# PimLb/POMDP_PBVI_Exploration

Hardware: AMD Instinct MI355X
Metric: alpha-vector backups/sec (higher is better)
Workload: dtype f32

## Files before the change

### pomdp_pbvi_exploration_amd/csrc/engine.hip

```cpp
#include <algorithm>
#include <cmath>
#include <cstdio>
#include <cstdlib>
#include <cstring>
#include <condition_variable>
#include <mutex>
#include <new>
#include <string>
#include <thread>
#include <unistd.h>
#include <vector>

#include "backup_kernels.h"

namespace pbvi {

static thread_local std::string g_err;
static int g_poison = -1;
static bool poison_enabled() {
    if (g_poison < 0) g_poison = getenv("PBVI_POISON") != nullptr ? 1 : 0;
    return g_poison == 1;
}
void set_error(const std::string& msg) { g_err = msg; }

#define HIPCHK(expr)                                                                         \
    do {                                                                                     \
        hipError_t _e = (expr);                                                              \
        if (_e != hipSuccess) {                                                              \
            set_error(std::string(#expr) + ": " + hipGetErrorString(_e));                    \
            (void)hipGetLastError();                                                         \
            return (_e == hipErrorOutOfMemory || _e == hipErrorMemoryAllocation) ? PBVI_ENOMEM : PBVI_ERUNTIME; \
        }                                                                                    \
    } while (0)

#define FAIL(code, msg)        \
    do {                       \
        set_error(msg);        \
        return (code);         \
    } while (0)

class CopyPool {
public:
    static CopyPool& get() {
        static CopyPool* pool = new CopyPool();
        return *pool;
    }
// ... 296 lines not shown
    for (int off = 32; off > 0; off >>= 1) {
        const int o = __shfl_xor(first, off, 64);
        first = o < first ? o : first;
    }
    if ((tid & 63) == 0) red[tid >> 6] = first;
    __syncthreads();
    if (tid == 0) {
        int m = red[0];
        for (int w = 1; w < 4; ++w) m = red[w] < m ? red[w] : m;
        key[b] = m == 0x7fffffff ? k_tiles : m;
    }
}

__global__ void k_rank_sort(const int32_t* __restrict__ key, int B, int32_t* __restrict__ perm) {
    const int lane = threadIdx.x & 63;
    const int i = blockIdx.x * 4 + (threadIdx.x >> 6);
    if (i >= B) return;
    const int ki = key[i];
    int rank = 0;
    for (int j = lane; j < B; j += 64) {
        const int kj = key[j];
        rank += (kj < ki || (kj == ki && j < i)) ? 1 : 0;
    }
#pragma unroll
    for (int off = 32; off > 0; off >>= 1) rank += __shfl_xor(rank, off, 64);
    if (lane == 0) perm[rank] = i;
}

__device__ __forceinline__ void tile_or_block(const uint8_t* __restrict__ flags, const int32_t* __restrict__ perm, int B, int k_tiles,
                                              uint8_t* __restrict__ nz, int bx, int tile);
template <typename T>
__global__ void k_gather_rows_v(const T* __restrict__ src, T* __restrict__ dst, int ld, const int32_t* __restrict__ perm,
                                const int32_t* __restrict__ ids, const uint8_t* __restrict__ flags = nullptr, int B = 0,
                                int k_tiles = 0, uint8_t* __restrict__ nz = nullptr, int or_rows = 0) {
    if ((int)blockIdx.y < or_rows) {
        if ((int)blockIdx.x * 64 < k_tiles) tile_or_block(flags, perm, B, k_tiles, nz, blockIdx.x, blockIdx.y);
        return;
    }
    constexpr int NS = 16 / (int)sizeof(T);
    typedef T TN __attribute__((ext_vector_type(NS)));
    const int c = blockIdx.x * 256 + threadIdx.x;
    if (c * NS >= ld) return;
    const int row = blockIdx.y - or_rows;
    int r = row;
    if (perm) r = perm[r];
    if (ids) r = ids[r];
    *(TN*)(dst + (int64_t)row * ld + (int64_t)c * NS) = *(const TN*)(src + (int64_t)r * ld + (int64_t)c * NS);
}

__device__ __forceinline__ void tile_or_block(const uint8_t* __restrict__ flags, const int32_t* __restrict__ perm, int B, int k_tiles,
                                              uint8_t* __restrict__ nz, int bx, int tile) {
    __shared__ uint32_t part[16][17];
    const int cw = threadIdx.x & 15, rs = threadIdx.x >> 4;
    const int kt0 = (bx * 16 + cw) * 4;
    const int r1 = (tile + 1) * 256 < B ? (tile + 1) * 256 : B;
    uint32_t f = 0;
    if (kt0 < k_tiles) {
        const bool whole = kt0 + 4 <= k_tiles && (k_tiles & 3) == 0;
#pragma unroll 4
        for (int r = tile * 256 + rs; r < r1; r += 16) {
            const uint8_t* p = flags + (int64_t)(perm ? perm[r] : r) * k_tiles + kt0;
            if (whole) {
                f |= *(const uint32_t*)p;
            } else {
                for (int e = 0; e < 4 && kt0 + e < k_tiles; ++e) f |= (uint32_t)p[e] << (8 * e);
            }
        }
    }
    part[rs][cw] = f;
    __syncthreads();
    if (rs == 0 && kt0 < k_tiles) {
        for (int x = 1; x < 16; ++x) f |= part[x][cw];
        for (int e = 0; e < 4 && kt0 + e < k_tiles; ++e) nz[(int64_t)tile * k_tiles + kt0 + e] = ((f >> (8 * e)) & 0xffu) ? 1 : 0;
    }
}

template <typename T>
__global__ void k_gather_rows(const T* __restrict__ src, T* __restrict__ dst, int ld, const int32_t* __restrict__ perm) {
    const int s = blockIdx.x * 256 + threadIdx.x;
    if (s >= ld) return;
// ... 190 lines not shown
};

template <typename T>
class EngineT : public EngineBase {
   public:
    static constexpr bool kF32 = sizeof(T) == 4;

    int device_ = 0;
    hipStream_t stream_ = nullptr;
    int S_ = 0, A_ = 0, O_ = 0, R_ = 0, S_pad_ = 0, mode_ = 0;
    int64_t bytes_ = 0;
    int64_t room() const {
        if (DevBuf::limit_bytes() >= 0) return DevBuf::limit_bytes() - bytes_;
        size_t fr = 0, tot = 0;
        if (hipMemGetInfo(&fr, &tot) != hipSuccess) {
            (void)hipGetLastError();
            return INT64_MAX;
        }
        return (int64_t)fr;
    }
    double tie_rel_user_ = -1.0;

    DevBuf rs_, rto_, er_, sup_;
    DevBuf alpha_, alpha_buf_, alpha_small_;
    std::vector<int32_t> prim_ids_;
    int64_t prim_off_ = 0;
    bool prim_valid_ = false, alpha_on_primary_ = false;
    uint64_t prim_layout_ver_ = 0;
    uint64_t screen_layout_seen_ = 0;
    int64_t screen_off_seen_ = 0;
    int64_t V_ = 0;
    DevBuf bel_;
    int64_t B_ = 0, B_pad_ = 0;
    DevBuf gam_, slabs_, best_v_, best_score_, err_, dead_, queue_, counters_, rdot_, action_, aqueue_, out_, keep_;
    DevBuf bv2_, bs2_, err2_, queue2_, prune_cnt_;
    DevBuf stage_, keys_, perm_, action_res_, best_res_;
    DevBuf rep_, uniq_, inv_, slot_, out_full_;
    DevBuf store_[2], ids_;
    int64_t store_rows_[2] = {0, 0};
    DevBuf in_ptr_, in_src_, bu_act_, bu_obs_, bu_row_, bu_unnorm_, bu_mass_, bu_out_, walk64_, rto64_;
    std::vector<int32_t> h_rs_;
    DevBuf btl_, btc_, val_exact_;
    DevBuf bp_, nzP_, pmag_, prd_;
    bool btl_valid_ = false;
    bool vmax_exact_ = true;
    DevBuf snz_, sbtl_, sbtc_;
    int64_t snz_rows_ = 0, sbt_rows_ = 0;
    int64_t walk_rows_ = 0;
    DevBuf vmax_bk_;
    bool have_bk_vmax_ = false;
    hipEvent_t walk_ev_[8] = {};
    void* host_stage_ = nullptr;
    size_t host_stage_cap_ = 0;
    DevBuf keys_tmp_, keys_act_, keys_best_, keys_rows_;
    DevBuf acand_;
    DevBuf rf_q2_, rf_q2p_, rf_q2d_;
    DevBuf rf_v_, rf_slot_, rf_sc_, rf_entry_, rf_n_, rf_tiles_, rf_ibv_, rf_ibi_, rf_cnt_, rf_W_, rf_Cx_, rf_nzW_, rf_klW_, rf_kcW_;
    int formulation_ = 0;
    int last_formulation_ = 1;
    int64_t f64_pairs_ = 0;
    const int32_t* res_action_ = nullptr;
    const int32_t* res_best_ = nullptr;
    int64_t res_unique_ = 0;
    bool full_valid_ = false;
    std::vector<int32_t> h_perm_;
    bool h_perm_valid_ = false;
// ... 36 lines not shown
    int64_t res_B_ = 0;
    int screen_mode_ = 1;
    int split_mode_ = 1;
    bool split_supported_ = false;
    int fuse_project_ = 1;
    double irr_frac_ = 0.0;
    DevBuf irr_;
    DevBuf mat_, vlist_;
    DevBuf ctile_;
    std::vector<int32_t> h_ctile_;
    int n_mat_ = 0;
    bool gam_pad_compact_ = false;
    std::vector<uint8_t> h_mat_;
    std::vector<int> h_vlist_;
    int64_t mat_V_ = -1;
    uint64_t dead_ver_ = 0;
    int64_t dead_pairs_ = 0, dead_count_ = 0;
    int* rf_counts_ = nullptr;
    bool last_deferred_nothing_ = false;
    bool owns_streams_ = true;
    EngineT<float>* screen_ = nullptr;
    std::vector<int32_t> h_reach_ref_;
    std::vector<double> h_rto_ref_, h_er_ref_;
    uint64_t alpha_ver_ = 1, bel_ver_ = 1;
    uint64_t screen_alpha_seen_ = 0, screen_bel_seen_ = 0;

    ~EngineT() override {
        (void)hipSetDevice(device_);
        if (screen_) {
            (void)hipStreamSynchronize(stream_);
            delete screen_;
            screen_ = nullptr;
        }
        DevBuf* all[] = {&rs_, &rto_, &er_, &sup_, &alpha_buf_, &alpha_small_, &bel_, &gam_, &slabs_, &best_v_, &best_score_, &err_,
                         &dead_, &queue_, &counters_, &rdot_, &action_, &aqueue_, &out_, &keep_, &bv2_, &bs2_,
                         &err2_, &queue2_, &prune_cnt_, &nzB_, &nzA_, &klist_, &kcount_, &nchunks_, &need_, &skws_, &stage_, &keys_, &perm_,
                         &action_res_, &best_res_, &rep_, &uniq_, &inv_, &slot_, &out_full_, &btl_, &btc_, &val_exact_, &store_[0], &store_[1], &ids_, &in_ptr_, &in_src_, &bu_act_, &bu_obs_,
                         &bu_unnorm_, &bu_mass_, &bu_out_, &bu_row_, &walk64_, &rto64_, &bp_, &nzP_, &pmag_, &prd_, &keys_tmp_, &keys_act_, &keys_best_, &keys_rows_, &rf_v_, &rf_slot_, &rf_sc_, &rf_entry_, &rf_n_, &rf_tiles_,
                         &snz_, &sbtl_, &sbtc_, &vmax_bk_, &rf_ibv_, &rf_ibi_, &rf_cnt_, &rf_W_, &rf_Cx_, &rf_nzW_, &rf_klW_, &rf_kcW_,
                         &dense_, &nzD_, &nzAlpha_, &prod_, &klistD_, &kcountD_, &nchunksD_, &mat_, &vlist_, &irr_, &rowflags_, &nzBw_, &scr_flag_, &ctile_, &acand_, &rf_q2_, &rf_q2p_, &rf_q2d_, &e_bv_, &e_bs_, &e_err_, &e_rdot_, &e_act_, &e_ares_, &e_bres_, &e_rep_, &e_uniq_, &e_inv_, &e_slotd_, &e_cnt_, &e_out_, &e_slot_};
        static const bool dbg = getenv("PBVI_DEBUG") != nullptr;
        auto chk = [&](hipError_t e, const char* what) {
            if (e != hipSuccess && dbg) fprintf(stderr, "[pbvi] engine teardown: %s: %s\n", what, hipGetErrorString(e));
        };
        for (auto& e : walk_ev_)
            if (e) chk(hipEventDestroy(e), "hipEventDestroy(walk)");
        for (DevBuf* b : all) b->release();
        if (host_stage_) chk(hipHostFree(host_stage_), "hipHostFree(stage)");
        if (ids_pin_) chk(hipHostFree(ids_pin_), "hipHostFree(ids)");
        if (h_flag_) chk(hipHostFree(h_flag_), "hipHostFree(flag)");
        if (kc_pin_) chk(hipHostFree(kc_pin_), "hipHostFree(kcount)");
        for (hipEvent_t& ev : ev_early_)
            if (ev) chk(hipEventDestroy(ev), "hipEventDestroy(early)");
        if (ev_ids_) chk(hipEventDestroy(ev_ids_), "hipEventDestroy(ids)");
        if (ev_nzA_) chk(hipEventDestroy(ev_nzA_), "hipEventDestroy(nzA)");
        for (auto& e : ev_)
            if (e) chk(hipEventDestroy(e), "hipEventDestroy(ev)");
        for (auto& e : ev_pg_)
            if (e) chk(hipEventDestroy(e), "hipEventDestroy(ev_pg)");
        if (ev_fork_) chk(hipEventDestroy(ev_fork_), "hipEventDestroy(fork)");
        if (ev_join_) chk(hipEventDestroy(ev_join_), "hipEventDestroy(join)");
        if (ev_lists_) chk(hipEventDestroy(ev_lists_), "hipEventDestroy(lists)");
        for (auto& e : ev_xr_)
            if (e) chk(hipEventDestroy(e), "hipEventDestroy(xr)");
        if (owns_streams_) {
            if (stream3_) chk(hipStreamDestroy(stream3_), "hipStreamDestroy(3)");
            if (stream2_) chk(hipStreamDestroy(stream2_), "hipStreamDestroy(2)");
// ... 257 lines not shown
                HIPCHK(hipMemcpyAsync(nb.p, alpha_.p, (size_t)V_ * S_pad_ * sizeof(T), hipMemcpyDeviceToDevice, stream_));
            HIPCHK(hipStreamSynchronize(stream_));
            bytes_ -= (int64_t)alpha_buf_.cap;
            alpha_buf_.release();
            alpha_buf_ = nb;
            alpha_view(alpha_buf_, 0);
        } else {
            HIPCHK(hipMemsetAsync(alpha_.as<T>() + (size_t)V_ * S_pad_, 0, (size_t)S_pad_ * sizeof(T), stream_));
        }
        prim_valid_ = alpha_on_primary_ = false;
        HIPCHK(hipMemcpy2DAsync(alpha_.as<T>() + (size_t)V_ * S_pad_, (size_t)S_pad_ * sizeof(T), alpha,
                                (size_t)S_ * sizeof(T), (size_t)S_ * sizeof(T), (size_t)n, hipMemcpyHostToDevice, stream_));
        V_ = Vn;
        ++alpha_ver_;
        int rc = refresh_magnitude_row();
        if (rc) return rc;
        HIPCHK(hipStreamSynchronize(stream_));
        have_result_ = false;
        return PBVI_OK;
    }

    int64_t alpha_count() const override { return V_; }

    int beliefs_finish(int64_t B, const T* src, const int32_t* src_ids) {
        const int64_t Bp = round_up(B, GEMM_BM);
        const int k_tiles = S_pad_ / GEMM_BK;
        int rc = bel_.ensure((size_t)Bp * S_pad_ * sizeof(T), &bytes_);
        if (rc) return rc;
        if ((rc = rowflags_.ensure((size_t)B * k_tiles, &bytes_))) return rc;
        if ((rc = keys_.ensure((size_t)B * sizeof(int32_t), &bytes_))) return rc;
        if ((rc = perm_.ensure((size_t)B * sizeof(int32_t), &bytes_))) return rc;
        if ((rc = nzA_.ensure((size_t)(Bp / GEMM_BM) * k_tiles, &bytes_))) return rc;
        if (Bp > B) HIPCHK(hipMemsetAsync(bel_.as<T>() + (size_t)B * S_pad_, 0, (size_t)(Bp - B) * S_pad_ * sizeof(T), stream_));
        static const bool no_sort = getenv("PBVI_NO_BELIEF_SORT") != nullptr;
        sorted_ = B > (kF32 ? GEMM_BM : 128) && !no_sort;
        hipLaunchKernelGGL(k_row_flags<T>, dim3((unsigned)B), dim3(256), 0, stream_, src, S_pad_, src_ids, S_pad_, k_tiles,
                           rowflags_.as<uint8_t>(), keys_.as<int32_t>());
        HIPCHK(hipGetLastError());
        const int32_t* perm = nullptr;
        if (sorted_) {
            hipLaunchKernelGGL(k_rank_sort, dim3((unsigned)((B + 3) / 4)), dim3(256), 0, stream_, keys_.as<int32_t>(), (int)B,
                               perm_.as<int32_t>());
            HIPCHK(hipGetLastError());
            perm = perm_.as<int32_t>();
        }
        constexpr int NS = 16 / (int)sizeof(T);
        const int or_rows = (int)(Bp / GEMM_BM);
        hipLaunchKernelGGL(k_gather_rows_v<T>, dim3((S_pad_ / NS + 255) / 256, (unsigned)(B + or_rows)), dim3(256), 0, stream_, src,
                           bel_.as<T>(), S_pad_, perm, src_ids, rowflags_.as<uint8_t>(), (int)B, k_tiles, nzA_.as<uint8_t>(), or_rows);
        HIPCHK(hipGetLastError());
        if (!ev_nzA_) HIPCHK(hipEventCreateWithFlags(&ev_nzA_, hipEventDisableTiming));
        HIPCHK(hipEventRecord(ev_nzA_, stream_));
        B_ = B;
        B_pad_ = Bp;
        ++bel_ver_;
        rowflags_ver_ = bel_ver_;
        nzA_ver_ = bel_ver_;
        h_perm_valid_ = false;
        have_result_ = false;
        btl_valid_ = false;
        return PBVI_OK;
    }

    int* pinned_flag() {
        if (!h_flag_ && hipHostMalloc((void**)&h_flag_, 128, hipHostMallocDefault) != hipSuccess) {
            (void)hipGetLastError();
            h_flag_ = nullptr;
        }
        return h_flag_;
    }

    int host_perm() {
        if (!sorted_ || h_perm_valid_) return PBVI_OK;
        h_perm_.resize((size_t)B_);
        HIPCHK(hipMemcpyAsync(h_perm_.data(), perm_.p, (size_t)B_ * sizeof(int32_t), hipMemcpyDeviceToHost, stream_));
        HIPCHK(hipStreamSynchronize(stream_));
        h_perm_valid_ = true;
        return PBVI_OK;
    }

    int beliefs_set(const void* bel, int64_t B) override {
        if (B <= 0 || bel == nullptr) FAIL(PBVI_EINVAL, "beliefs_set: need B > 0 and a non-null array");
        if (B > 65535) FAIL(PBVI_EUNSUPPORTED, "beliefs_set: at most 65535 beliefs per block");
        HIPCHK(hipSetDevice(device_));
        int rc = stage_.ensure((size_t)B * S_pad_ * sizeof(T), &bytes_);
        if (rc) return rc;
        HIPCHK(hipMemsetAsync(stage_.p, 0, (size_t)B * S_pad_ * sizeof(T), stream_));
        HIPCHK(hipMemcpy2DAsync(stage_.p, (size_t)S_pad_ * sizeof(T), bel, (size_t)S_ * sizeof(T), (size_t)S_ * sizeof(T),
                                (size_t)B, hipMemcpyHostToDevice, stream_));
        if ((rc = beliefs_finish(B, stage_.as<T>(), nullptr))) return rc;
// ... 300 lines not shown
        walk_rows_ = n;
        return first;
    }

    int backup_value_max(double* out_value) override {
        if (!have_result_ || !have_bk_vmax_)
            FAIL(PBVI_EUNSUPPORTED, "backup_fetch_value_max: the last backup did not run in the belief-side formulation");
        if (!out_value) FAIL(PBVI_EINVAL, "backup_fetch_value_max: NULL destination");
        HIPCHK(hipSetDevice(device_));
        int rc;
        if ((rc = out_begin())) return rc;
        if ((rc = out_add(out_value, vmax_bk_.p, (size_t)res_B_ * sizeof(double)))) return rc;
        return out_finish();
    }

    int walk_keys(int64_t n, uint64_t* out_keys) override {
        if (n <= 0 || n != walk_rows_ || !out_keys) FAIL(PBVI_EINVAL, "belief_walk_keys: n must be the length of the last walk");
        HIPCHK(hipSetDevice(device_));
        int rc = keys_tmp_.ensure((size_t)n * sizeof(uint64_t), &bytes_);
        if (rc) return rc;
        hipLaunchKernelGGL(k_row_hash<double>, dim3((unsigned)n), dim3(256), 0, stream_, walk64_.as<double>() + S_, S_, S_,
                           keys_tmp_.as<unsigned long long>());
        HIPCHK(hipGetLastError());
        if ((rc = out_begin())) return rc;
        if ((rc = out_add(out_keys, keys_tmp_.p, (size_t)n * sizeof(uint64_t)))) return rc;
        return out_finish();
    }

    int after_oom() override {
        HIPCHK(hipSetDevice(device_));
        (void)hipStreamSynchronize(stream_);
        if (stream2_) (void)hipStreamSynchronize(stream2_);
        if (stream3_) (void)hipStreamSynchronize(stream3_);
        DevBuf* drop[] = {&alpha_buf_, &alpha_small_, &bel_, &gam_, &slabs_, &best_v_, &best_score_, &err_, &dead_, &queue_, &rdot_,
                          &action_, &aqueue_, &out_, &keep_, &bv2_, &bs2_, &err2_, &queue2_, &prune_cnt_, &nzA_, &klist_, &kcount_,
                          &nchunks_, &need_, &skws_, &stage_, &keys_, &perm_, &action_res_, &best_res_, &rep_, &uniq_, &inv_, &slot_,
                          &out_full_, &btl_, &btc_, &val_exact_, &store_[0], &store_[1], &ids_, &bu_act_, &bu_obs_, &bu_unnorm_,
                          &bu_mass_, &bu_out_, &bu_row_, &walk64_, &bp_, &nzP_, &pmag_, &prd_, &keys_tmp_, &keys_act_, &keys_best_,
                          &keys_rows_, &rf_v_, &rf_slot_, &rf_sc_, &rf_entry_, &rf_n_, &rf_tiles_, &snz_, &sbtl_, &sbtc_, &vmax_bk_,
                          &rf_ibv_, &rf_ibi_, &rf_cnt_, &rf_W_, &rf_Cx_, &rf_nzW_, &rf_klW_, &rf_kcW_, &nzAlpha_, &prod_, &klistD_,
                          &kcountD_, &nchunksD_, &mat_, &vlist_, &rowflags_, &ctile_, &acand_, &rf_q2_, &rf_q2p_, &rf_q2d_, &e_bv_, &e_bs_, &e_err_, &e_rdot_, &e_act_, &e_ares_, &e_bres_, &e_rep_, &e_uniq_, &e_inv_, &e_slotd_, &e_out_, &e_slot_};
        for (DevBuf* b : drop) {
            bytes_ -= (int64_t)b->cap;
            b->release();
        }
        alpha_ = DevBuf{};
        V_ = 0;
        B_ = B_pad_ = 0;
        prim_valid_ = alpha_on_primary_ = false;
        prim_ids_.clear();
        prim_off_ = 0;
        store_rows_[0] = store_rows_[1] = 0;
        snz_rows_ = sbt_rows_ = 0;
        walk_rows_ = 0;
        have_result_ = have_bk_vmax_ = false;
        btl_valid_ = false;
        sorted_ = false;
        h_perm_valid_ = false;
        mat_V_ = -1;
        gam_pad_ptr_ = nullptr;
        last_deferred_nothing_ = false;
        ++alpha_ver_;
        ++bel_ver_;
        if (screen_) {
            screen_alpha_seen_ = screen_bel_seen_ = 0;
            screen_layout_seen_ = 0;
            return screen_->after_oom();
        }
        return PBVI_OK;
    }

    int store_reset(int which) override {
        if (which < 0 || which > 1) FAIL(PBVI_EINVAL, "store_reset: bad store");
        store_rows_[which] = 0;
        if (which == 1) snz_rows_ = sbt_rows_ = 0;
        if (which == 0) {
            prim_valid_ = false;
            prim_ids_.clear();
        }
        return PBVI_OK;
    }

    int store_select(int which, const int32_t* ids, int64_t n) override {
        if (which < 0 || which > 1 || n <= 0 || ids == nullptr) FAIL(PBVI_EINVAL, "store_select: bad arguments");
        if (n > 65535 && which == 1) FAIL(PBVI_EUNSUPPORTED, "at most 65535 beliefs per block");
        for (int64_t i = 0; i < n; ++i)
            if (ids[i] < 0 || ids[i] >= store_rows_[which]) FAIL(PBVI_EINVAL, "store_select: id out of range");
        HIPCHK(hipSetDevice(device_));
        int rc = ids_.ensure((size_t)n * sizeof(int32_t), &bytes_);
        if (rc) return rc;
        if (which == 1) {
            const size_t bytes = (size_t)n * sizeof(int32_t);
            if (ids_pin_cap_ < bytes) {
                HIPCHK(hipStreamSynchronize(stream_));
                if (ids_pin_) (void)hipHostFree(ids_pin_);
                ids_pin_ = nullptr;
// ... 593 lines not shown
        int64_t w_slots = std::min<int64_t>(std::min<int64_t>(slots, 65535),
                                            ((int64_t)2 << 30) / ((int64_t)S_pad_ * sizeof(double)));
        if (const char* c = getenv("PBVI_REFINE_DEFER_MIN")) w->defer_min = atoi(c);
        if (const char* c = getenv("PBVI_REFINE_W_SLOTS")) w_slots = std::min<int64_t>(slots, std::max<int64_t>(0, atoll(c)));
        if (w_slots > 0) {
            if ((rc = build_inverse_lists())) return rc;
            const int kt32 = S_pad_ / GEMM_BK;
            if ((rc = rf_W_.ensure((size_t)w_slots * S_pad_ * sizeof(double), &bytes_))) return rc;
            if ((rc = rf_Cx_.ensure((size_t)w_slots * V * sizeof(double), &bytes_))) return rc;
            if ((rc = rf_nzW_.ensure((size_t)((w_slots + 255) / 256) * kt32, &bytes_))) return rc;
            if ((rc = rf_klW_.ensure(gemm_f64_klist_ints((int)w_slots, (int)V, kt32) * sizeof(int), &bytes_))) return rc;
            if ((rc = rf_kcW_.ensure(gemm_f64_kcount_ints((int)w_slots, (int)V, kt32) * sizeof(int), &bytes_))) return rc;
            w->W = rf_W_.as<double>();
            w->Cx = rf_Cx_.as<double>();
            w->nzW = rf_nzW_.as<uint8_t>();
            w->klistW = rf_klW_.as<int>();
            w->kcountW = rf_kcW_.as<int>();
            w->in_ptr = in_ptr_.as<int32_t>();
            w->in_src = in_src_.as<int32_t>();
        }
        w->w_slot_cap = (int)w_slots;
        return PBVI_OK;
    }

    bool vmax_skinny() const {
        static const bool off = getenv("PBVI_NO_SKINNY") != nullptr;
        return kF32 && !off && V_ > 0 && V_ <= 64 && mode_ == PBVI_SPARSE;
    }
    static constexpr int64_t kSplitMinSteps = 16384;
    bool split_pays(int64_t n_rows_alloc, int k_tiles) const {
        const int64_t dense_steps = (B_pad_ / GEMM_BM) * (n_rows_alloc / GEMM_BN) * (int64_t)k_tiles;
        return dense_steps >= kSplitMinSteps;
    }
    static bool f64_uses_mfma(int64_t m_rows, int64_t n_rows) {
        static const bool simple = getenv("PBVI_F64_SIMPLE") != nullptr;
        return !simple && m_rows * n_rows >= 64 * 64;
    }

    int set_fused(int enable) override {
        fuse_project_ = enable < 0 ? 0 : (enable > 2 ? 2 : enable);
        if (screen_) screen_->fuse_project_ = fuse_project_;
        return PBVI_OK;
    }
    int set_screen(int mode) override {
        if (mode < 0 || mode > 2) FAIL(PBVI_EINVAL, "set_f64_screen: 0 = never, 1 = automatic, 2 = always");
        screen_mode_ = mode;
        return PBVI_OK;
    }
    int set_score_split(int mode) override {
        if (mode < 0 || mode > 2) FAIL(PBVI_EINVAL, "set_score_split: 0 = never, 1 = automatic, 2 = always");
        split_mode_ = mode;
        return PBVI_OK;
    }
    int set_formulation(int f) override {
        if (f < 0 || f > 2) FAIL(PBVI_EINVAL, "set_formulation: 0 = auto, 1 = project alpha-vectors, 2 = project beliefs");
        formulation_ = f;
        return PBVI_OK;
    }
    int set_value_max_exact(int exact) override {
        vmax_exact_ = exact != 0;
        return PBVI_OK;
    }
    int alpha_layout(int64_t* free_rows, int64_t* layouts) override {
        if (free_rows) *free_rows = alpha_on_primary_ ? prim_off_ : 0;
        if (layouts) *layouts = (int64_t)prim_layout_ver_;
        return alpha_on_primary_ ? 1 : 0;
    }

    int set_tie_window(double rel) override {
        tie_rel_user_ = rel;
        return PBVI_OK;
    }
    int64_t device_bytes() const override { return bytes_ + (screen_ ? screen_->bytes_ : 0); }
};

template <typename T>
int EngineT<T>::score_gemm(const T* Y, int64_t rows_y, const uint8_t* nzB, int G, int v_group, SlabView<T>* sv,
                           const T* X, int64_t x_rows, const uint8_t* nzX, hipStream_t list_stream, const FusedB* fused,
                           int* split) {
    int rc;
    const int64_t m_rows = X ? x_rows : B_;
    const int64_t m_pad = X ? round_up(x_rows, GEMM_BM) : B_pad_;
    if (!X) {
        X = bel_.as<T>();
        nzX = nzA_.as<uint8_t>();
    }
    if constexpr (kF32) {
        const int64_t n_pad = round_up(rows_y, GEMM_BN);
        if (m_pad > 0x7fffffff || n_pad > 0x7fffffff) FAIL(PBVI_EUNSUPPORTED, "score_gemm: operand rows exceed int32");
        plan_ = make_gemm_plan((int)m_pad, (int)n_pad, S_pad_);
        const size_t pairs = (size_t)plan_.tiles_m * plan_.tiles_n;
        if ((rc = slabs_.ensure((size_t)plan_.c_floats * sizeof(float), &bytes_))) return rc;
        if ((rc = klist_.ensure(pairs * plan_.k_tiles * sizeof(int), &bytes_))) return rc;
        if ((rc = kcount_.ensure(pairs * sizeof(int), &bytes_))) return rc;
        if ((rc = nchunks_.ensure(pairs * sizeof(int), &bytes_))) return rc;
        if ((rc = skws_.ensure(streamk_workspace_ints(plan_) * sizeof(int), &bytes_))) return rc;
        const int sp = split != nullptr && *split && plan_.streamk && (fused == nullptr || fused->R == 1) ? 1 : 0;
        if (split != nullptr) *split = sp;
        HIPCHK(launch_gemm_nt_f32((const float*)X, S_pad_, (const float*)Y, S_pad_, slabs_.as<float>(), plan_,
                                  nzX, nzB, G, v_group, (int)rows_y, klist_.as<int>(), kcount_.as<int>(),
                                  nchunks_.as<int>(), stream_, 1, 0, 0, skws_.as<int>(), list_stream, ev_lists_, nullptr, nullptr,
                                  fused, sp));
        sv->slabs = slabs_.as<T>();
        sv->slab_stride = plan_.slab_stride;
        sv->ldc = plan_.ldc;
        sv->nchunks = nchunks_.as<int>();
        sv->tiles_m = plan_.tiles_m;
        sv->fixed = 0;
        sv->first_block = plan_.streamk ? skws_.as<int>() + (pairs + 1) + plan_.nblocks : nullptr;
    } else {
        const int kt32s = S_pad_ / GEMM_BK;
        const int split = f64_uses_mfma(m_rows, rows_y) ? gemm_f64_split((int)m_rows, (int)rows_y, kt32s) : 1;
        if ((rc = slabs_.ensure((size_t)split * m_rows * rows_y * sizeof(T), &bytes_))) return rc;
        f64_pairs_ = 0;
        if (!f64_uses_mfma(m_rows, rows_y)) {
            HIPCHK(launch_gemm_nt_simple<T>(X, S_pad_, Y, S_pad_, slabs_.as<T>(), (int)rows_y, (int)m_rows, (int)rows_y,
                                            S_, stream_));
        } else {
            const int kt32 = S_pad_ / GEMM_BK;
            if ((rc = klist_.ensure(gemm_f64_klist_ints((int)m_rows, (int)rows_y, kt32) * sizeof(int), &bytes_))) return rc;
            if ((rc = kcount_.ensure(gemm_f64_kcount_ints((int)m_rows, (int)rows_y, kt32) * sizeof(int), &bytes_))) return rc;
            HIPCHK(launch_gemm_nt_f64((const double*)X, S_pad_, (int)m_rows, (const double*)Y, S_pad_, (int)rows_y,
                                      slabs_.as<double>(), (int)rows_y, S_pad_, nzX, nzB, G, v_group, klist_.as<int>(),
                                      kcount_.as<int>(), stream_, split, m_rows * rows_y));
            f64_pairs_ = (int64_t)gemm_f64_pairs((int)m_rows, (int)rows_y);
        }
        sv->slabs = slabs_.as<T>();
        sv->slab_stride = 0;
        sv->ldc = (int)rows_y;
        sv->nchunks = nullptr;
        sv->tiles_m = 0;
        sv->fixed = 1;
// ... 1295 lines not shown
```

### pomdp_pbvi_exploration_amd/csrc/gemm.hip

```cpp
#include "pbvi_common.h"

#include <cstdlib>
#include <map>
#include <mutex>

namespace pbvi {

typedef float f32x4 __attribute__((ext_vector_type(4)));
typedef float f32x16 __attribute__((ext_vector_type(16)));

constexpr int TILE_FLOATS = 256 * GEMM_BK;
constexpr int KL_IRR_BIT = 30;
constexpr int KL_MASK = (1 << KL_IRR_BIT) - 1;
constexpr int GEMM_LDS_BYTES = 4 * TILE_FLOATS * 4;

__device__ __forceinline__ void glds16(const float* g, float* l) {
    __builtin_amdgcn_global_load_lds((const __attribute__((address_space(1))) void*)g,
                                     (__attribute__((address_space(3))) void*)l, 16, 0, 0);
}

struct TileThread {
    int lane, wid, i, h, wr, wc;
    int srow[4], scol[4];
    int a_row[4], b_row[2];
    __device__ __forceinline__ void init() {
        const int tid = threadIdx.x;
        lane = tid & 63;
        wid = __builtin_amdgcn_readfirstlane(tid >> 6);
        i = lane & 31;
        h = lane >> 5;
        wr = wid >> 2;
        wc = wid & 3;
#pragma unroll
// ... 577 lines not shown
            ++p;
            continue;
        }
        const int u_lo = (int)(pos - prefix[p]);
        const int64_t room = end - pos;
        const int u_hi = (u_lo + room < cnt + ovh) ? (int)(u_lo + room) : cnt + ovh;
        const int lo = u_lo > ovh ? u_lo - ovh : 0;
        const int hi = u_hi > ovh ? u_hi - ovh : 0;
        if (hi > lo) {
            const int tm = p % tiles_m, tn = p / tiles_m;
            f32x16 acc[4][2];
            tile_zero(acc);
            if (fb.mat[tn]) {
                tile_run(t, lds, A + (int64_t)tm * 256 * lda, lda, B + (int64_t)tn * 256 * ldb, ldb,
                         klist + (int64_t)p * k_tiles, lo, hi, acc);
            } else {
                const int r0 = tn * 256;
                const int g = r0 / fb.V, v0 = r0 - g * fb.V;
                tile_run_fused_r<R>(t, lds, A + (int64_t)tm * 256 * lda, lda, B + (int64_t)tn * 256 * ldb, ldb,
                                 fb.rs + (int64_t)(g / fb.O) * R * fb.S_pad, fb.rto + (int64_t)g * R * fb.S_pad,
                                 fb.S_pad, fb.alpha + (int64_t)(v0 + t.srow[0]) * fb.lda, (int64_t)64 * fb.lda, fb.gamma,
                                 klist + (int64_t)p * k_tiles, lo, hi, acc);
            }
            const bool cont = L != first_block[p];
            tile_store(t, cont ? C + slab_stride + (int64_t)L * (256 * 256) : C, cont ? 256 : ldc, cont ? 0 : tm, cont ? 0 : tn, acc);
        }
        pos += u_hi - u_lo;
        ++p;
    }
}

typedef __bf16 bf16x8 __attribute__((ext_vector_type(8)));

__device__ __forceinline__ uint32_t cvt_pk_bf16(float a, float b) {
    uint32_t r;
    asm("v_cvt_pk_bf16_f32 %0, %1, %2" : "=v"(r) : "v"(a), "v"(b));
    return r;
}
__device__ __forceinline__ float bf16_sat(float x) {
    const float m = 0x1.fep127f;
    return fabsf(x) > m ? copysignf(m, x) : x;
}
__device__ __forceinline__ void split_pair(float x0, float x1, uint32_t& hi, uint32_t& lo) {
#pragma clang fp contract(off)
    hi = cvt_pk_bf16(bf16_sat(x0), bf16_sat(x1));
    const float h0 = __uint_as_float(hi << 16), h1 = __uint_as_float(hi & 0xffff0000u);
    lo = cvt_pk_bf16(x0 - h0, x1 - h1);
}
__device__ __forceinline__ void split_store(float* lop, int row, int kg, const f32x4& x0, const f32x4& x1) {
    i32x4 hi, lo;
    uint32_t h, l;
    split_pair(x0[0], x0[1], h, l); hi[0] = (int)h; lo[0] = (int)l;
    split_pair(x0[2], x0[3], h, l); hi[1] = (int)h; lo[1] = (int)l;
    split_pair(x1[0], x1[1], h, l); hi[2] = (int)h; lo[2] = (int)l;
    split_pair(x1[2], x1[3], h, l); hi[3] = (int)h; lo[3] = (int)l;
    const int sw = (row >> 1) & 7;
    *(i32x4*)(lop + row * GEMM_BK + (kg ^ sw) * 4) = hi;
    *(i32x4*)(lop + row * GEMM_BK + ((4 + kg) ^ sw) * 4) = lo;
}

__device__ __forceinline__ void split_compute(const TileThread& t, const float* lds, int buf, f32x16 (&acc)[4][2]) {
    const float* la = lds + buf * 2 * TILE_FLOATS;
    const float* lb = la + TILE_FLOATS;
#pragma unroll
    for (int kk = 0; kk < 2; ++kk) {
        i32x4 ah[4], al[4], bh[2], bl[2];
#pragma unroll
        for (int mi = 0; mi < 4; ++mi) {
            const int r = t.a_row[mi], sw = (r >> 1) & 7;
            ah[mi] = *(const i32x4*)(la + r * GEMM_BK + ((2 * kk + t.h) ^ sw) * 4);
            al[mi] = *(const i32x4*)(la + r * GEMM_BK + ((4 + 2 * kk + t.h) ^ sw) * 4);
        }
#pragma unroll
        for (int ni = 0; ni < 2; ++ni) {
            const int r = t.b_row[ni], sw = (r >> 1) & 7;
            bh[ni] = *(const i32x4*)(lb + r * GEMM_BK + ((2 * kk + t.h) ^ sw) * 4);
            bl[ni] = *(const i32x4*)(lb + r * GEMM_BK + ((4 + 2 * kk + t.h) ^ sw) * 4);
        }
#pragma unroll
        for (int term = 0; term < 3; ++term)
#pragma unroll
            for (int mi = 0; mi < 4; ++mi)
#pragma unroll
                for (int ni = 0; ni < 2; ++ni) {
                    const i32x4 a = term == 2 ? al[mi] : ah[mi];
                    const i32x4 b = term == 1 ? bl[ni] : bh[ni];
                    acc[mi][ni] = __builtin_amdgcn_mfma_f32_32x32x16_bf16(__builtin_bit_cast(bf16x8, a), __builtin_bit_cast(bf16x8, b),
                                                                          acc[mi][ni], 0, 0, 0);
                }
    }
}

__device__ __forceinline__ void tile_run_split(const TileThread& t, float* lds, const float* Ablk, int lda, const float* Bblk,
                                               int ldb, bool gen, const int32_t* __restrict__ rsrow,
                                               const float* __restrict__ rtorow, const float* __restrict__ arow0,
                                               int64_t a_step, float gamma, const int* __restrict__ kl, int i0, int i1,
                                               f32x16 (&acc)[4][2]) {
    const int tid = threadIdx.x;
    const int kg = tid & 3, r0 = tid >> 2;
    f32x4 xa[2][2], xb[2][2];
    i32x4 idx[2];
    f32x4 w[2];
    auto load_rows = [&](f32x4 (&x)[2][2], const float* base, int ld, int entry) {
        const int k = (entry & KL_MASK) * GEMM_BK + kg * 8;
#pragma unroll
        for (int it = 0; it < 2; ++it) {
            const float* p = base + (int64_t)(it * 128 + r0) * ld + k;
            ld16(x[it][0], p);
            ld16(x[it][1], p + 4);
        }
    };
    auto tables = [&](int entry) {
        const int s = (entry & KL_MASK) * GEMM_BK + kg * 8;
        ld16i(idx[0], rsrow + s);
        ld16i(idx[1], rsrow + s + 4);
        ld16(w[0], rtorow + s);
        ld16(w[1], rtorow + s + 4);
    };
    auto alphas = [&](int entry) {
        if (entry >> KL_IRR_BIT) {
#pragma unroll
            for (int it = 0; it < 2; ++it) {
                const float* arow = arow0 + it * a_step;
#pragma unroll
                for (int q = 0; q < 2; ++q) {
                    float e0, e1, e2, e3;
                    ld4(e0, arow + idx[q][0]);
                    ld4(e1, arow + idx[q][1]);
                    ld4(e2, arow + idx[q][2]);
                    ld4(e3, arow + idx[q][3]);
                    asm volatile("s_waitcnt vmcnt(0)\n\tv_mov_b32 %0, %4\n\tv_mov_b32 %1, %5\n\tv_mov_b32 %2, %6\n\tv_mov_b32 %3, %7"
                                 : "=&v"(xb[it][q].x), "=&v"(xb[it][q].y), "=&v"(xb[it][q].z), "=&v"(xb[it][q].w)
                                 : "v"(e0), "v"(e1), "v"(e2), "v"(e3)
                                 : "memory");
                }
            }
        } else {
#pragma unroll
            for (int it = 0; it < 2; ++it) {
                ld16(xb[it][0], arow0 + it * a_step + idx[0][0]);
                ld16(xb[it][1], arow0 + it * a_step + idx[1][0]);
            }
        }
    };
    auto store = [&](int buf) {
        float* la = lds + buf * 2 * TILE_FLOATS;
        float* lb = la + TILE_FLOATS;
#pragma unroll
        for (int it = 0; it < 2; ++it) {
            split_store(la, it * 128 + r0, kg, xa[it][0], xa[it][1]);
            if (gen)
                split_store(lb, it * 128 + r0, kg, fused_value(gamma, w[0], xb[it][0]), fused_value(gamma, w[1], xb[it][1]));
            else
                split_store(lb, it * 128 + r0, kg, xb[it][0], xb[it][1]);
        }
    };
    auto wait_all = [&]() {
        asm volatile("s_waitcnt vmcnt(0)"
                     : "+v"(xa[0][0]), "+v"(xa[0][1]), "+v"(xa[1][0]), "+v"(xa[1][1]), "+v"(xb[0][0]), "+v"(xb[0][1]),
                       "+v"(xb[1][0]), "+v"(xb[1][1])::"memory");
    };
    {
        const int e0 = kl[i0];
        if (gen) {
            tables(e0);
            asm volatile("s_waitcnt vmcnt(0)" : "+v"(idx[0]), "+v"(idx[1]), "+v"(w[0]), "+v"(w[1])::"memory");
            alphas(e0);
        } else {
            load_rows(xb, Bblk, ldb, e0);
        }
        load_rows(xa, Ablk, lda, e0);
        wait_all();
        store(0);
    }
    int k_next = (i0 + 1 < i1) ? kl[i0 + 1] : 0;
    __syncthreads();
    int buf = 0;
    for (int it = i0; it < i1; ++it) {
        int k_after = 0;
        const bool more = it + 1 < i1;
        if (more) {
            if (gen) tables(k_next);
            load_rows(xa, Ablk, lda, k_next);
            if (!gen) load_rows(xb, Bblk, ldb, k_next);
            if (it + 2 < i1) k_after = kl[it + 2];
        }
        split_compute(t, lds, buf, acc);
        if (more) {
            if (gen) {
                asm volatile("s_waitcnt vmcnt(4)" : "+v"(idx[0]), "+v"(idx[1]), "+v"(w[0]), "+v"(w[1])::"memory");
                alphas(k_next);
            }
            wait_all();
            store(buf ^ 1);
        }
        __syncthreads();
        buf ^= 1;
        k_next = k_after;
    }
}

__global__ __launch_bounds__(512) void k_gemm_split_streamk(
    const float* __restrict__ A, int lda, const float* __restrict__ B, int ldb, FusedB fb, float* __restrict__ C, int ldc,
    int64_t slab_stride, int tiles_m, int pairs, int k_tiles, const int* __restrict__ klist, const int* __restrict__ kcount,
    const int* __restrict__ prefix, const int* __restrict__ start_pair, const int* __restrict__ first_block,
    const int* __restrict__ plan, int ovh) {
    extern __shared__ __attribute__((aligned(16))) float lds[];
    const int nb = gridDim.x;
    int L;
    {
        const int bid = blockIdx.x, xcd = bid & 7, qq = nb >> 3, r = nb & 7;
        const int base = (xcd < r) ? xcd * (qq + 1) : r * (qq + 1) + (xcd - r) * qq;
        L = base + (bid >> 3);
    }
    const int q = plan[0], T = plan[1];
    int64_t pos = (int64_t)L * q;
    if (pos >= T) return;
    const int64_t end = (pos + q < T) ? pos + q : T;
    int p = start_pair[L];
    if (p < 0) return;
    TileThread t;
    t.init();
    while (pos < end && p < pairs) {
        const int cnt = kcount[p];
        if (cnt == 0) {
            ++p;
            continue;
        }
        const int u_lo = (int)(pos - prefix[p]);
        const int64_t room = end - pos;
        const int u_hi = (u_lo + room < cnt + ovh) ? (int)(u_lo + room) : cnt + ovh;
// ... 365 lines not shown
```

Measured before the change: 636,900.

## Pre-split belief matrix into bf16 hi/lo plane and stage it via direct LDS loads

```diff
diff --git a/pomdp_pbvi_exploration_amd/csrc/engine.hip b/pomdp_pbvi_exploration_amd/csrc/engine.hip
--- a/pomdp_pbvi_exploration_amd/csrc/engine.hip
+++ b/pomdp_pbvi_exploration_amd/csrc/engine.hip
@@ -12,6 +12,7 @@
 #include <vector>
 
 #include "backup_kernels.h"
+#include "split_bf16.h"
 
 namespace pbvi {
 
@@ -374,7 +375,8 @@
 template <typename T>
 __global__ void k_gather_rows_v(const T* __restrict__ src, T* __restrict__ dst, int ld, const int32_t* __restrict__ perm,
                                 const int32_t* __restrict__ ids, const uint8_t* __restrict__ flags = nullptr, int B = 0,
-                                int k_tiles = 0, uint8_t* __restrict__ nz = nullptr, int or_rows = 0) {
+                                int k_tiles = 0, uint8_t* __restrict__ nz = nullptr, int or_rows = 0,
+                                uint32_t* __restrict__ plane = nullptr) {
     if ((int)blockIdx.y < or_rows) {
         if ((int)blockIdx.x * 64 < k_tiles) tile_or_block(flags, perm, B, k_tiles, nz, blockIdx.x, blockIdx.y);
         return;
@@ -387,7 +389,28 @@
     int r = row;
     if (perm) r = perm[r];
     if (ids) r = ids[r];
-    *(TN*)(dst + (int64_t)row * ld + (int64_t)c * NS) = *(const TN*)(src + (int64_t)r * ld + (int64_t)c * NS);
+    const TN v = *(const TN*)(src + (int64_t)r * ld + (int64_t)c * NS);
+    *(TN*)(dst + (int64_t)row * ld + (int64_t)c * NS) = v;
+    if constexpr (NS == 4) {
+        if (plane != nullptr) {
+            uint2 hi, lo;
+            split_quad(v[0], v[1], v[2], v[3], hi, lo);
+            uint32_t* pw = plane + (int64_t)row * ld + (c >> 3) * GEMM_BK + 2 * (c & 7);
+            *(uint2*)pw = hi;
+            *(uint2*)(pw + 16) = lo;
+        }
+    }
+}
+
+__global__ void k_split_plane(const float* __restrict__ x, uint32_t* __restrict__ plane, int64_t n) {
+    const int64_t c = (int64_t)blockIdx.x * 256 + threadIdx.x;
+    if (c * 4 >= n) return;
+    const float4 v = *(const float4*)(x + c * 4);
+    uint2 hi, lo;
+    split_quad(v.x, v.y, v.z, v.w, hi, lo);
+    uint32_t* pw = plane + (c >> 3) * GEMM_BK + 2 * (c & 7);
+    *(uint2*)pw = hi;
+    *(uint2*)(pw + 16) = lo;
 }
 
 __device__ __forceinline__ void tile_or_block(const uint8_t* __restrict__ flags, const int32_t* __restrict__ perm, int B, int k_tiles,
@@ -644,6 +667,8 @@
     int64_t V_ = 0;
     DevBuf bel_;
     int64_t B_ = 0, B_pad_ = 0;
+    DevBuf belsp_;
+    uint64_t belsp_ver_ = 0;
     DevBuf gam_, slabs_, best_v_, best_score_, err_, dead_, queue_, counters_, rdot_, action_, aqueue_, out_, keep_;
     DevBuf bv2_, bs2_, err2_, queue2_, prune_cnt_;
     DevBuf stage_, keys_, perm_, action_res_, best_res_;
@@ -746,7 +771,7 @@
             delete screen_;
             screen_ = nullptr;
         }
-        DevBuf* all[] = {&rs_, &rto_, &er_, &sup_, &alpha_buf_, &alpha_small_, &bel_, &gam_, &slabs_, &best_v_, &best_score_, &err_,
+        DevBuf* all[] = {&rs_, &rto_, &er_, &sup_, &alpha_buf_, &alpha_small_, &bel_, &belsp_, &gam_, &slabs_, &best_v_, &best_score_, &err_,
                          &dead_, &queue_, &counters_, &rdot_, &action_, &aqueue_, &out_, &keep_, &bv2_, &bs2_,
                          &err2_, &queue2_, &prune_cnt_, &nzB_, &nzA_, &klist_, &kcount_, &nchunks_, &need_, &skws_, &stage_, &keys_, &perm_,
                          &action_res_, &best_res_, &rep_, &uniq_, &inv_, &slot_, &out_full_, &btl_, &btc_, &val_exact_, &store_[0], &store_[1], &ids_, &in_ptr_, &in_src_, &bu_act_, &bu_obs_,
@@ -1070,6 +1095,11 @@
         if ((rc = perm_.ensure((size_t)B * sizeof(int32_t), &bytes_))) return rc;
         if ((rc = nzA_.ensure((size_t)(Bp / GEMM_BM) * k_tiles, &bytes_))) return rc;
         if (Bp > B) HIPCHK(hipMemsetAsync(bel_.as<T>() + (size_t)B * S_pad_, 0, (size_t)(Bp - B) * S_pad_ * sizeof(T), stream_));
+        uint32_t* plane = nullptr;
+        if (kF32 && split_mode_ != 0 && split_supported_ && belsp_.cap >= (size_t)Bp * S_pad_ * sizeof(float)) {
+            plane = belsp_.as<uint32_t>();
+            if (Bp > B) HIPCHK(hipMemsetAsync(plane + (size_t)B * S_pad_, 0, (size_t)(Bp - B) * S_pad_ * sizeof(float), stream_));
+        }
         static const bool no_sort = getenv("PBVI_NO_BELIEF_SORT") != nullptr;
         sorted_ = B > (kF32 ? GEMM_BM : 128) && !no_sort;
         hipLaunchKernelGGL(k_row_flags<T>, dim3((unsigned)B), dim3(256), 0, stream_, src, S_pad_, src_ids, S_pad_, k_tiles,
@@ -1085,7 +1115,8 @@
         constexpr int NS = 16 / (int)sizeof(T);
         const int or_rows = (int)(Bp / GEMM_BM);
         hipLaunchKernelGGL(k_gather_rows_v<T>, dim3((S_pad_ / NS + 255) / 256, (unsigned)(B + or_rows)), dim3(256), 0, stream_, src,
-                           bel_.as<T>(), S_pad_, perm, src_ids, rowflags_.as<uint8_t>(), (int)B, k_tiles, nzA_.as<uint8_t>(), or_rows);
+                           bel_.as<T>(), S_pad_, perm, src_ids, rowflags_.as<uint8_t>(), (int)B, k_tiles, nzA_.as<uint8_t>(), or_rows,
+                           plane);
         HIPCHK(hipGetLastError());
         if (!ev_nzA_) HIPCHK(hipEventCreateWithFlags(&ev_nzA_, hipEventDisableTiming));
         HIPCHK(hipEventRecord(ev_nzA_, stream_));
@@ -1094,6 +1125,7 @@
         ++bel_ver_;
         rowflags_ver_ = bel_ver_;
         nzA_ver_ = bel_ver_;
+        belsp_ver_ = plane != nullptr ? bel_ver_ : 0;
         h_perm_valid_ = false;
         have_result_ = false;
         btl_valid_ = false;
@@ -1460,7 +1492,7 @@
         (void)hipStreamSynchronize(stream_);
         if (stream2_) (void)hipStreamSynchronize(stream2_);
         if (stream3_) (void)hipStreamSynchronize(stream3_);
-        DevBuf* drop[] = {&alpha_buf_, &alpha_small_, &bel_, &gam_, &slabs_, &best_v_, &best_score_, &err_, &dead_, &queue_, &rdot_,
+        DevBuf* drop[] = {&alpha_buf_, &alpha_small_, &bel_, &belsp_, &gam_, &slabs_, &best_v_, &best_score_, &err_, &dead_, &queue_, &rdot_,
                           &action_, &aqueue_, &out_, &keep_, &bv2_, &bs2_, &err2_, &queue2_, &prune_cnt_, &nzA_, &klist_, &kcount_,
                           &nchunks_, &need_, &skws_, &stage_, &keys_, &perm_, &action_res_, &best_res_, &rep_, &uniq_, &inv_, &slot_,
                           &out_full_, &btl_, &btc_, &val_exact_, &store_[0], &store_[1], &ids_, &bu_act_, &bu_obs_, &bu_unnorm_,
@@ -1490,6 +1522,7 @@
         last_deferred_nothing_ = false;
         ++alpha_ver_;
         ++bel_ver_;
+        belsp_ver_ = 0;
         if (screen_) {
             screen_alpha_seen_ = screen_bel_seen_ = 0;
             screen_layout_seen_ = 0;
@@ -2149,6 +2182,22 @@
         const int64_t dense_steps = (B_pad_ / GEMM_BM) * (n_rows_alloc / GEMM_BN) * (int64_t)k_tiles;
         return dense_steps >= kSplitMinSteps;
     }
+    bool split_plane() {
+        const size_t bytes = (size_t)B_pad_ * S_pad_ * sizeof(float);
+        if (bytes == 0 || S_pad_ > (1 << 22)) return false;
+        if (belsp_.cap < bytes) {
+            if (!DevBuf::headroom_ok(bytes_, bytes) || belsp_.ensure(bytes, &bytes_) != PBVI_OK) return false;
+            belsp_ver_ = 0;
+        }
+        if (belsp_ver_ != bel_ver_) {
+            const int64_t n = (int64_t)B_pad_ * S_pad_;
+            hipLaunchKernelGGL(k_split_plane, dim3((unsigned)((n / 4 + 255) / 256)), dim3(256), 0, stream_, bel_.as<float>(),
+                               belsp_.as<uint32_t>(), n);
+            if (hipGetLastError() != hipSuccess) return false;
+            belsp_ver_ = bel_ver_;
+        }
+        return true;
+    }
     static bool f64_uses_mfma(int64_t m_rows, int64_t n_rows) {
         static const bool simple = getenv("PBVI_F64_SIMPLE") != nullptr;
         return !simple && m_rows * n_rows >= 64 * 64;
@@ -2198,6 +2247,7 @@
     int rc;
     const int64_t m_rows = X ? x_rows : B_;
     const int64_t m_pad = X ? round_up(x_rows, GEMM_BM) : B_pad_;
+    const bool own_block = X == nullptr;
     if (!X) {
         X = bel_.as<T>();
         nzX = nzA_.as<uint8_t>();
@@ -2212,9 +2262,10 @@
         if ((rc = kcount_.ensure(pairs * sizeof(int), &bytes_))) return rc;
         if ((rc = nchunks_.ensure(pairs * sizeof(int), &bytes_))) return rc;
         if ((rc = skws_.ensure(streamk_workspace_ints(plan_) * sizeof(int), &bytes_))) return rc;
-        const int sp = split != nullptr && *split && plan_.streamk && (fused == nullptr || fused->R == 1) ? 1 : 0;
+        int sp = split != nullptr && *split && plan_.streamk && (fused == nullptr || fused->R == 1) ? 1 : 0;
+        if (sp && (!own_block || !split_plane())) sp = 0;
         if (split != nullptr) *split = sp;
-        HIPCHK(launch_gemm_nt_f32((const float*)X, S_pad_, (const float*)Y, S_pad_, slabs_.as<float>(), plan_,
+        HIPCHK(launch_gemm_nt_f32(sp ? belsp_.as<float>() : (const float*)X, S_pad_, (const float*)Y, S_pad_, slabs_.as<float>(), plan_,
                                   nzX, nzB, G, v_group, (int)rows_y, klist_.as<int>(), kcount_.as<int>(),
                                   nchunks_.as<int>(), stream_, 1, 0, 0, skws_.as<int>(), list_stream, ev_lists_, nullptr, nullptr,
                                   fused, sp));
diff --git a/pomdp_pbvi_exploration_amd/csrc/gemm.hip b/pomdp_pbvi_exploration_amd/csrc/gemm.hip
--- a/pomdp_pbvi_exploration_amd/csrc/gemm.hip
+++ b/pomdp_pbvi_exploration_amd/csrc/gemm.hip
@@ -1,4 +1,5 @@
 #include "pbvi_common.h"
+#include "split_bf16.h"
 
 #include <cstdlib>
 #include <map>
@@ -642,21 +643,6 @@
 
 typedef __bf16 bf16x8 __attribute__((ext_vector_type(8)));
 
-__device__ __forceinline__ uint32_t cvt_pk_bf16(float a, float b) {
-    uint32_t r;
-    asm("v_cvt_pk_bf16_f32 %0, %1, %2" : "=v"(r) : "v"(a), "v"(b));
-    return r;
-}
-__device__ __forceinline__ float bf16_sat(float x) {
-    const float m = 0x1.fep127f;
-    return fabsf(x) > m ? copysignf(m, x) : x;
-}
-__device__ __forceinline__ void split_pair(float x0, float x1, uint32_t& hi, uint32_t& lo) {
-#pragma clang fp contract(off)
-    hi = cvt_pk_bf16(bf16_sat(x0), bf16_sat(x1));
-    const float h0 = __uint_as_float(hi << 16), h1 = __uint_as_float(hi & 0xffff0000u);
-    lo = cvt_pk_bf16(x0 - h0, x1 - h1);
-}
 __device__ __forceinline__ void split_store(float* lop, int row, int kg, const f32x4& x0, const f32x4& x1) {
     i32x4 hi, lo;
     uint32_t h, l;
@@ -669,61 +655,75 @@
     *(i32x4*)(lop + row * GEMM_BK + ((4 + kg) ^ sw) * 4) = lo;
 }
 
-__device__ __forceinline__ void split_compute(const TileThread& t, const float* lds, int buf, f32x16 (&acc)[4][2]) {
+struct SplitFrag {
+    i32x4 ah[4], al[4], bh[2], bl[2];
+};
+__device__ __forceinline__ void split_group(const TileThread& t, const float* lds, int buf, int kk, int term, SplitFrag& f,
+                                            f32x16 (&acc)[4][2]) {
     const float* la = lds + buf * 2 * TILE_FLOATS;
     const float* lb = la + TILE_FLOATS;
-#pragma unroll
-    for (int kk = 0; kk < 2; ++kk) {
-        i32x4 ah[4], al[4], bh[2], bl[2];
+    const int hc = 2 * kk + t.h;
+    if (term != 1) {
 #pragma unroll
         for (int mi = 0; mi < 4; ++mi) {
             const int r = t.a_row[mi], sw = (r >> 1) & 7;
-            ah[mi] = *(const i32x4*)(la + r * GEMM_BK + ((2 * kk + t.h) ^ sw) * 4);
-            al[mi] = *(const i32x4*)(la + r * GEMM_BK + ((4 + 2 * kk + t.h) ^ sw) * 4);
-        }
+            if (term == 0) f.ah[mi] = *(const i32x4*)(la + r * GEMM_BK + (hc ^ sw) * 4);
+            else f.al[mi] = *(const i32x4*)(la + r * GEMM_BK + ((4 + hc) ^ sw) * 4);
+        }
+    }
+    if (term != 2) {
 #pragma unroll
         for (int ni = 0; ni < 2; ++ni) {
             const int r = t.b_row[ni], sw = (r >> 1) & 7;
-            bh[ni] = *(const i32x4*)(lb + r * GEMM_BK + ((2 * kk + t.h) ^ sw) * 4);
-            bl[ni] = *(const i32x4*)(lb + r * GEMM_BK + ((4 + 2 * kk + t.h) ^ sw) * 4);
-        }
-#pragma unroll
-        for (int term = 0; term < 3; ++term)
-#pragma unroll
-            for (int mi = 0; mi < 4; ++mi)
-#pragma unroll
-                for (int ni = 0; ni < 2; ++ni) {
-                    const i32x4 a = term == 2 ? al[mi] : ah[mi];
-                    const i32x4 b = term == 1 ? bl[ni] : bh[ni];
-                    acc[mi][ni] = __builtin_amdgcn_mfma_f32_32x32x16_bf16(__builtin_bit_cast(bf16x8, a), __builtin_bit_cast(bf16x8, b),
-                                                                          acc[mi][ni], 0, 0, 0);
-                }
-    }
-}
-
-__device__ __forceinline__ void tile_run_split(const TileThread& t, float* lds, const float* Ablk, int lda, const float* Bblk,
+            if (term == 0) f.bh[ni] = *(const i32x4*)(lb + r * GEMM_BK + (hc ^ sw) * 4);
+            else f.bl[ni] = *(const i32x4*)(lb + r * GEMM_BK + ((4 + hc) ^ sw) * 4);
+        }
+    }
+#pragma unroll
+    for (int mi = 0; mi < 4; ++mi)
+#pragma unroll
+        for (int ni = 0; ni < 2; ++ni) {
+            const i32x4 a = term == 2 ? f.al[mi] : f.ah[mi];
+            const i32x4 b = term == 1 ? f.bl[ni] : f.bh[ni];
+            acc[mi][ni] = __builtin_amdgcn_mfma_f32_32x32x16_bf16(__builtin_bit_cast(bf16x8, a), __builtin_bit_cast(bf16x8, b),
+                                                                  acc[mi][ni], 0, 0, 0);
+        }
+}
+
+__device__ __forceinline__ void tile_run_split(const TileThread& t, float* lds, const float* Aplane, int lda, const float* Bblk,
                                                int ldb, bool gen, const int32_t* __restrict__ rsrow,
                                                const float* __restrict__ rtorow, const float* __restrict__ arow0,
                                                int64_t a_step, float gamma, const int* __restrict__ kl, int i0, int i1,
                                                f32x16 (&acc)[4][2]) {
     const int tid = threadIdx.x;
     const int kg = tid & 3, r0 = tid >> 2;
-    f32x4 xa[2][2], xb[2][2];
+    f32x4 xb[2][2];
     i32x4 idx[2];
     f32x4 w[2];
-    auto load_rows = [&](f32x4 (&x)[2][2], const float* base, int ld, int entry) {
+    const uint32_t a_off = (uint32_t)(t.srow[0] * lda + t.scol[0]) * 4u;
+    auto stage_a = [&](int buf, int entry) {
+        const char* base = (const char*)(Aplane + (int64_t)(entry & KL_MASK) * GEMM_BK);
+        float* la = lds + buf * 2 * TILE_FLOATS;
+#pragma unroll
+        for (int it = 0; it < 4; ++it)
+            glds16((const float*)(base + (int64_t)it * 64 * lda * 4 + a_off), la + (it * 512 + t.wid * 64) * 4);
+    };
+    auto load_rows = [&](int entry) {
         const int k = (entry & KL_MASK) * GEMM_BK + kg * 8;
 #pragma unroll
         for (int it = 0; it < 2; ++it) {
-            const float* p = base + (int64_t)(it * 128 + r0) * ld + k;
-            ld16(x[it][0], p);
-            ld16(x[it][1], p + 4);
-        }
-    };
-    auto tables = [&](int entry) {
+            const float* p = Bblk + (int64_t)(it * 128 + r0) * ldb + k;
+            ld16(xb[it][0], p);
+            ld16(xb[it][1], p + 4);
+        }
+    };
+    auto indices = [&](int entry) {
         const int s = (entry & KL_MASK) * GEMM_BK + kg * 8;
         ld16i(idx[0], rsrow + s);
         ld16i(idx[1], rsrow + s + 4);
+    };
+    auto weights = [&](int entry) {
+        const int s = (entry & KL_MASK) * GEMM_BK + kg * 8;
         ld16(w[0], rtorow + s);
         ld16(w[1], rtorow + s + 4);
     };
@@ -753,60 +753,69 @@
             }
         }
     };
-    auto store = [&](int buf) {
-        float* la = lds + buf * 2 * TILE_FLOATS;
-        float* lb = la + TILE_FLOATS;
-#pragma unroll
-        for (int it = 0; it < 2; ++it) {
-            split_store(la, it * 128 + r0, kg, xa[it][0], xa[it][1]);
-            if (gen)
-                split_store(lb, it * 128 + r0, kg, fused_value(gamma, w[0], xb[it][0]), fused_value(gamma, w[1], xb[it][1]));
-            else
-                split_store(lb, it * 128 + r0, kg, xb[it][0], xb[it][1]);
-        }
-    };
-    auto wait_all = [&]() {
-        asm volatile("s_waitcnt vmcnt(0)"
-                     : "+v"(xa[0][0]), "+v"(xa[0][1]), "+v"(xa[1][0]), "+v"(xa[1][1]), "+v"(xb[0][0]), "+v"(xb[0][1]),
-                       "+v"(xb[1][0]), "+v"(xb[1][1])::"memory");
+    auto store_b = [&](int buf, int it) {
+        float* lb = lds + buf * 2 * TILE_FLOATS + TILE_FLOATS;
+        if (gen)
+            split_store(lb, it * 128 + r0, kg, fused_value(gamma, w[0], xb[it][0]), fused_value(gamma, w[1], xb[it][1]));
+        else
+            split_store(lb, it * 128 + r0, kg, xb[it][0], xb[it][1]);
     };
     {
         const int e0 = kl[i0];
         if (gen) {
-            tables(e0);
-            asm volatile("s_waitcnt vmcnt(0)" : "+v"(idx[0]), "+v"(idx[1]), "+v"(w[0]), "+v"(w[1])::"memory");
+            indices(e0);
+            weights(e0);
+            asm volatile("s_waitcnt vmcnt(0)" : "+v"(idx[0]), "+v"(idx[1])::"memory");
             alphas(e0);
+            indices(i0 + 1 < i1 ? kl[i0 + 1] : 0);
         } else {
-            load_rows(xb, Bblk, ldb, e0);
-        }
-        load_rows(xa, Ablk, lda, e0);
-        wait_all();
-        store(0);
+            load_rows(e0);
+        }
+        stage_a(0, e0);
+        asm volatile("s_waitcnt vmcnt(0)" : "+v"(xb[0][0]), "+v"(xb[0][1]), "+v"(xb[1][0]), "+v"(xb[1][1]), "+v"(w[0]), "+v"(w[1]),
+                     "+v"(idx[0]), "+v"(idx[1])::"memory");
+        store_b(0, 0);
+        store_b(0, 1);
     }
     int k_next = (i0 + 1 < i1) ? kl[i0 + 1] : 0;
+    int k_after = (i0 + 2 < i1) ? kl[i0 + 2] : 0;
     __syncthreads();
     int buf = 0;
     for (int it = i0; it < i1; ++it) {
-        int k_after = 0;
+        int k_after2 = 0;
         const bool more = it + 1 < i1;
         if (more) {
-            if (gen) tables(k_next);
-            load_rows(xa, Ablk, lda, k_next);
-            if (!gen) load_rows(xb, Bblk, ldb, k_next);
-            if (it + 2 < i1) k_after = kl[it + 2];
-        }
-        split_compute(t, lds, buf, acc);
+            if (gen) {
+                alphas(k_next);
+                weights(k_next);
+                indices(k_after);
+            } else {
+                load_rows(k_next);
+            }
+            stage_a(buf ^ 1, k_next);
+            if (it + 3 < i1) k_after2 = kl[it + 3];
+        }
+        SplitFrag f;
+        split_group(t, lds, buf, 0, 0, f, acc);
+        split_group(t, lds, buf, 0, 1, f, acc);
+        split_group(t, lds, buf, 0, 2, f, acc);
+        split_group(t, lds, buf, 1, 0, f, acc);
         if (more) {
-            if (gen) {
-                asm volatile("s_waitcnt vmcnt(4)" : "+v"(idx[0]), "+v"(idx[1]), "+v"(w[0]), "+v"(w[1])::"memory");
-                alphas(k_next);
-            }
-            wait_all();
-            store(buf ^ 1);
-        }
+            if (gen)
+                asm volatile("s_waitcnt vmcnt(6)" : "+v"(xb[0][0]), "+v"(xb[0][1]), "+v"(xb[1][0]), "+v"(xb[1][1]), "+v"(w[0]),
+                             "+v"(w[1])::"memory");
+            else
+                asm volatile("s_waitcnt vmcnt(4)" : "+v"(xb[0][0]), "+v"(xb[0][1]), "+v"(xb[1][0]), "+v"(xb[1][1])::"memory");
+            store_b(buf ^ 1, 0);
+        }
+        split_group(t, lds, buf, 1, 1, f, acc);
+        if (more) store_b(buf ^ 1, 1);
+        split_group(t, lds, buf, 1, 2, f, acc);
+        asm volatile("s_waitcnt vmcnt(0)" : "+v"(idx[0]), "+v"(idx[1])::"memory");
         __syncthreads();
         buf ^= 1;
         k_next = k_after;
+        k_after = k_after2;
     }
 }
 
diff --git a/pomdp_pbvi_exploration_amd/csrc/split_bf16.h b/pomdp_pbvi_exploration_amd/csrc/split_bf16.h
--- /dev/null
+++ b/pomdp_pbvi_exploration_amd/csrc/split_bf16.h
@@ -0,0 +1,28 @@
+#pragma once
+#include <hip/hip_runtime.h>
+#include <stdint.h>
+
+namespace pbvi {
+
+__device__ __forceinline__ uint32_t cvt_pk_bf16(float a, float b) {
+    uint32_t r;
+    asm("v_cvt_pk_bf16_f32 %0, %1, %2" : "=v"(r) : "v"(a), "v"(b));
+    return r;
+}
+__device__ __forceinline__ float bf16_sat(float x) {
+    const float m = 0x1.fep127f;
+    return fabsf(x) > m ? copysignf(m, x) : x;
+}
+__device__ __forceinline__ void split_pair(float x0, float x1, uint32_t& hi, uint32_t& lo) {
+#pragma clang fp contract(off)
+    hi = cvt_pk_bf16(bf16_sat(x0), bf16_sat(x1));
+    const float h0 = __uint_as_float(hi << 16), h1 = __uint_as_float(hi & 0xffff0000u);
+    lo = cvt_pk_bf16(x0 - h0, x1 - h1);
+}
+
+__device__ __forceinline__ void split_quad(float x0, float x1, float x2, float x3, uint2& hi, uint2& lo) {
+    split_pair(x0, x1, hi.x, lo.x);
+    split_pair(x2, x3, hi.y, lo.y);
+}
+
+}
```

Measured after the change: 654,100 (median of 6 runs). +2.7%, better.
